# angela000/DQNFlappyBird

Hardware: NVIDIA B200
Metric: env frames/sec (step+render+preproc) (higher is better)
Workload: dtype u8

## Files before the change

### dqnflappybird_b200/csrc/fb_qnet_tc.cu

```cuda
#include <cudaTypedefs.h>

#include <stdlib.h>
#include <string.h>

#include <map>
#include <new>
#include <vector>

#include "fb_qnet.cuh"
#include "fb_pack.cuh"
#include "fb_tc.cuh"
#include "fb_tc_conv.cuh"


namespace {

constexpr int kStages = 4;
constexpr int kMaxKb = 32;
constexpr int kG1 = 21, kP1 = 441;
constexpr int kG2 = 7, kP2 = 49;
constexpr int kThreads = 192;

struct GemmParams {
    int nkb, kper;
// ... 1783 lines not shown
    FinalizeArgs fa{t->part1, t->part2, t->part3, p->s1, p->s2, p->s3, t->bp1, t->bp2, t->bp3, c1, c23, c23, t->hp, t->hb, G, a.loss_out, 1.f / gscale};
    const int n_compact = L.wf1 + (L.total - L.bf1);
    const int nb_fin = (n_compact + 31) / 32;
    tc::pdl_next_launch_plain(t->nopdl & 16);
    FB_CUDA_OK(tc::launch_pdl(finalize_grads_kernel, dim3(nb_fin), dim3(32 * kFinWarps), 0, st, fa, L, a.grads, ad, t->pw[0]));
    if (a.ad.on && a.xch != nullptr) {
        rc = dist_launch_bucket(a.xch, n, 1, const_cast<float *>(a.params), a.ad.m, a.ad.v, t->adam_pow + 2, a.ad.beta1, a.ad.beta2, a.ad.eps,
                                a.ad.grad_scale, st);
        if (rc) return rc;
    }
    if (a.ad.on) FB_CUDA_OK(fork(t->aux3, st));
    if (per_on_side) FB_CUDA_OK(fork(t->aux4, st));
    return FB_OK;
}

bool same_key(const GraphKey &x, const GraphKey &y) { return memcmp(&x, &y, sizeof(GraphKey)) == 0; }

}

int tc_set_format(fb_qnet *n, int f16) {
    TcState *t = n->tc;
    FB_REQUIRE(t != nullptr, "tc_set_format: no tensor-core state");
    f16 = f16 ? 1 : 0;
    if (t->f16 != f16) {
        for (auto &g : t->graphs) destroy_entry(g);
        t->graphs.clear();
        t->plans.clear();
        n->packed_src[0] = n->packed_src[1] = nullptr;
    }
    t->f16 = f16; t->pw[0].f16 = f16; t->pw[1].f16 = f16;
    return FB_OK;
}

int tc_drop_graphs(fb_qnet *n) {
    if (n->tc) { for (auto &g : n->tc->graphs) destroy_entry(g); n->tc->graphs.clear(); }
    return FB_OK;
}

extern "C" int fb_qnet_set_conv1_mode(fb_qnet *n, int mode) {
    FB_REQUIRE(n != nullptr && n->tc != nullptr && mode >= 0 && mode <= 4, "fb_qnet_set_conv1_mode: needs a tensor-core precision and mode 0..4");
    n->tc->conv1_mode = mode;
    for (auto &g : n->tc->graphs) destroy_entry(g);
    n->tc->graphs.clear();
    return FB_OK;
}

extern "C" int fb_qnet_set_fused_backward(fb_qnet *n, int on) {
    FB_REQUIRE(n != nullptr && n->tc != nullptr, "fb_qnet_set_fused_backward: needs FB_PRECISION_BF16");
    n->tc->fuse_bwd = (on & 1) ? 1 : 0;
    n->tc->fuse_fwd = (on & 2) || on == 1 ? 1 : 0;
    return tc_drop_graphs(n);
}

extern "C" int fb_qnet_use_graphs(fb_qnet *n, int enable) {
    FB_REQUIRE(n != nullptr, "fb_qnet_use_graphs: NULL argument");
    if (n->tc) n->tc->use_graph = enable ? 1 : 0;
    return FB_OK;
}

int tc_step(fb_qnet *n, const QnetStep &a, float beta1_power, float beta2_power, cudaStream_t st) {
    TcState *t = n->tc;
    if (a.ad.on) {
        if (t->pow_host[0] != beta1_power || t->pow_host[1] != beta2_power) {
            float *slot = t->pow_pinned + 2 * (t->pow_slot++ & 15);
            slot[0] = beta1_power; slot[1] = beta2_power;
            FB_CUDA_OK(cudaMemcpyAsync(t->adam_pow, slot, 2 * sizeof(float), cudaMemcpyHostToDevice, st));
        }
        t->pow_host[0] = t->pow_host[1] = -1.f;
    }
    GraphKey key;
    memset(&key, 0, sizeof(key));
    memcpy(&key.a, &a, sizeof(a));
    key.a.pro.t = 0; key.a.pro.beta = 0.0;
    key.pack_online = n->packed_src[0] != a.params;
    key.pack_target = a.variant != 0 && n->packed_src[1] != a.target;
    int rc = FB_OK;
    GraphEntry *ge = nullptr;
    if (t->use_graph) {
        for (auto &g : t->graphs) if (same_key(g.key, key)) { ge = &g; break; }
        if (!ge) {
            if (t->graphs.size() >= 8) { for (auto &g : t->graphs) destroy_entry(g); t->graphs.clear(); }
            t->graphs.push_back(GraphEntry{key, 0, nullptr, nullptr, nullptr, nullptr});
            ge = &t->graphs.back();
        }
    }
    if (ge && ge->exec) {
        if (a.pro.replay != nullptr) { rc = replay_patch_nodes(ge->exec, ge->n_sampler, ge->n_gather, a.pro, a.gamma); if (rc) return rc; }
        FB_CUDA_OK(cudaGraphLaunch(ge->exec, st));
    } else if (ge && ge->seen >= 1) {
        cudaGraph_t graph = nullptr;
        FB_CUDA_OK(cudaStreamBeginCapture(t->cap, cudaStreamCaptureModeRelaxed));
        rc = train_step_launch(n, a, key.pack_online, key.pack_target, t->cap);
        cudaError_t ce = cudaStreamEndCapture(t->cap, &graph);
        if (rc) { if (graph) cudaGraphDestroy(graph); return rc; }
        FB_CUDA_OK(ce);
        cudaError_t ie = cudaGraphInstantiate(&ge->exec, graph, 0);
        if (ie == cudaSuccess && a.pro.replay != nullptr) {
            size_t nn = 0;
            cudaGraphGetNodes(graph, nullptr, &nn);
            std::vector<cudaGraphNode_t> nodes(nn);
            if (nn) cudaGraphGetNodes(graph, nodes.data(), &nn);
            for (size_t i = 0; i < nn; i++) {
                cudaGraphNodeType ty;
                if (cudaGraphNodeGetType(nodes[i], &ty) != cudaSuccess || ty != cudaGraphNodeTypeKernel) continue;
                cudaKernelNodeParams kp{};
                if (cudaGraphKernelNodeGetParams(nodes[i], &kp) != cudaSuccess) continue;
                if (replay_is_sampler(kp.func)) ge->n_sampler = nodes[i];
                else if (replay_is_gather(kp.func)) ge->n_gather = nodes[i];
            }
            if (!ge->n_sampler || !ge->n_gather) { cudaGraphExecDestroy(ge->exec); ge->exec = nullptr; ie = cudaErrorUnknown; }
        }
        if (ie == cudaSuccess && a.pro.replay != nullptr) ge->graph = graph;
        else cudaGraphDestroy(graph);
        FB_CUDA_OK(ie);
        FB_CUDA_OK(cudaGraphLaunch(ge->exec, st));
    } else {
        rc = train_step_launch(n, a, key.pack_online, key.pack_target, st);
        if (rc) return rc;
        if (ge) ge->seen++;
    }
    n->packed_src[0] = a.params;
    if (a.variant != 0) n->packed_src[1] = a.target;
    if (a.ad.on && n->packed_src[1] == a.params) n->packed_src[1] = nullptr;
    if (a.ad.on) { t->pow_host[0] = beta1_power * a.ad.beta1; t->pow_host[1] = beta2_power * a.ad.beta2; }
    return FB_OK;
}

extern "C" int fb_debug_tc_kernel(fb_qnet *n, int which, int B, int reps, const float *params_dev, void *stream) {
    FB_REQUIRE(n && n->tc && params_dev && B > 0 && B <= n->max_batch && reps > 0, "fb_debug_tc_kernel: bad argument");
    TcState *t = n->tc;
    TcPlan *p;
    int rc = make_plan(n, B, &p);
    if (rc) return rc;
    cudaStream_t st = (cudaStream_t)stream;
    const QnetLayout &L = n->L;
    const TcWeightMaps &wm = t->wm[0];
    const FwdWs &f = t->ws[0];
    const int H = L.hidden, P1 = B * kP1, P2 = B * kP2;
    for (int r = 0; r < reps; r++) {
        switch (which) {
            case 0: FB_CUDA_OK((launch_tc_conv<32, kSlab1, 1, 4, 6, 1>(p->x2_s[0], wm.w1p, p->conv1, t->n_sms, EpiConv1{f.z1, params_dev + L.b1, P1, t->f16}, st))); break;
            case 1: FB_CUDA_OK((launch_tc_conv<64, kSlab2, 2, 8, 3, 1>(p->p2_s[0], wm.w2p, p->conv2, t->n_sms, EpiGrid7{f.a2, params_dev + L.b2, P2, t->f16}, st))); break;
            case 2: FB_CUDA_OK((launch_tc_conv<64, kSlab3, 1, 9, 4, 1>(p->a2_s[0], wm.w3p, p->conv3, t->n_sms, EpiConv3{f.a3, params_dev + L.b3, P2, t->f16}, st))); break;
            case 3: FB_CUDA_OK((launch_tc_gemm<128, 2>(p->a3_k[0], wm.wf1n, p->fc1, dim3((B + 127) / 128, H / 128, p->sf),
                                                       EpiStoreF32{f.parth, B, H, (size_t)n->max_batch * H}, st))); break;
            case 4: FB_CUDA_OK((launch_tc_wgrad<32, 2, kSlabW1, 1, 6>(p->x2_w, p->dz1_b, p->conv1_w, p->s1, EpiStoreF32{t->part1, 256, 32, (size_t)256 * 32}, st))); break;
            case 5: FB_CUDA_OK((launch_tc_conv<64, kSlab3, 1, 9, 4, 1>(p->dz3_s, wm.w3d, p->conv3_d, t->n_sms, EpiConv3Dgrad{t->dz2, f.a2, P2, t->f16}, st))); break;
            case 6: FB_CUDA_OK((launch_tc_gemm<64, 0>(p->dh1_k, wm.wf1n, p->fc1_d, dim3((B + 127) / 128, kFlat / 64, 1), EpiFc1Dgrad{t->dz3, f.a3, B, t->f16}, st))); break;
            case 7: FB_CUDA_OK((launch_tc_conv1_fused<4, false>(p->x2_s[0], wm.w1p, Conv1FusedParams{g_probe_view, B, params_dev + L.b1, nullptr, f.p2, t->f16}, t->n_sms, st))); break;
            case 8: FB_CUDA_OK((launch_tc_conv1_fused<4, false>(p->x2_s[0], wm.w1p, Conv1FusedParams{g_probe_view, B, params_dev + L.b1, f.z1, f.p2, t->f16}, t->n_sms, st))); break;
            case 9: FB_CUDA_OK((launch_tc_conv1_fused<6, true>(p->x2_s[0], wm.w1p, Conv1FusedParams{g_probe_view, B, params_dev + L.b1, nullptr, f.p2, t->f16}, t->n_sms, st))); break;
            case 10: FB_CUDA_OK((launch_tc_conv1_fused<6, true>(p->x2_s[0], wm.w1p, Conv1FusedParams{g_probe_view, B, params_dev + L.b1, f.z1, f.p2, t->f16}, t->n_sms, st))); break;
            case 11: FB_CUDA_OK((launch_tc_conv1_fused<6, true>(p->x2_s[0], wm.w1p, Conv1FusedParams{g_probe_view, B, params_dev + L.b1, nullptr, nullptr, t->f16}, t->n_sms, st))); break;
            default: FB_REQUIRE(false, "fb_debug_tc_kernel: which must be 0..11");
        }
    }
    return FB_OK;
}

namespace {
__global__ void __launch_bounds__(128) tc_slab_probe_kernel(const __grid_constant__ CUtensorMap mapA, const __grid_constant__ CUtensorMap mapB,
                                                            int shift, uint32_t base_offset, float *d) {
    extern __shared__ uint8_t smem_raw[];
    __shared__ __align__(8) uint64_t bar_full, bar_done;
    __shared__ uint32_t tmem_slot;
    const uint32_t smem = (tc::smem_u32(smem_raw) + 1023u) & ~1023u;
    const int warp = threadIdx.x >> 5, lane = threadIdx.x & 31;
    if (threadIdx.x == 0) { tc::mbar_init(tc::smem_u32(&bar_full), 1); tc::mbar_init(tc::smem_u32(&bar_done), 1); tc::fence_barrier_init(); }
    if (warp == 0) tc::tmem_alloc(tc::smem_u32(&tmem_slot), 64);
    tc::tc_fence_before(); __syncthreads(); tc::tc_fence_after();
    const uint32_t tmem = tmem_slot, sa = smem, sb = smem + 32768;
    if (threadIdx.x == 0) {
        tc::mbar_expect_tx(tc::smem_u32(&bar_full), 32768 + 8192);
        tc::tma_load_2d(sa, &mapA, 0, 0, tc::smem_u32(&bar_full));
        tc::tma_load_2d(sa + 16384, &mapA, 0, 128, tc::smem_u32(&bar_full));
        tc::tma_load_2d(sb, &mapB, 0, 0, tc::smem_u32(&bar_full));
        tc::mbar_wait(tc::smem_u32(&bar_full), 0);
        tc::tc_fence_after();
        constexpr uint32_t idesc = tc::instr_desc_bf16(128, 64, 0, 0);
        for (int k = 0; k < 4; k++) {
            uint64_t ad = tc::smem_desc(sa + shift * 128 + k * 32, 16, 1024, tc::kSwizzle128) | ((uint64_t)(base_offset & 7u) << 49);
            uint64_t bd = tc::smem_desc(sb + k * 32, 16, 1024, tc::kSwizzle128);
            tc::umma_bf16(tmem, ad, bd, idesc, k != 0);
        }
        tc::umma_commit(tc::smem_u32(&bar_done));
    }
    tc::mbar_wait(tc::smem_u32(&bar_done), 0);
    tc::tc_fence_after();
    for (int c0 = 0; c0 < 64; c0 += 16) {
        float v[16];
        tc::tmem_ld16(tmem + ((uint32_t)(warp * 32) << 16) + (uint32_t)c0, v);
        for (int i = 0; i < 16; i++) d[(warp * 32 + lane) * 64 + c0 + i] = v[i];
    }
    tc::tc_fence_before(); __syncthreads();
    if (warp == 0) tc::tmem_dealloc(tmem, 64);
}
}

extern "C" int fb_debug_tc_slab(int shift, int base_offset, const void *a_dev, const void *b_dev, float *d_dev, void *stream) {
    FB_REQUIRE(a_dev && b_dev && d_dev && shift >= 0 && shift <= 128, "fb_debug_tc_slab: bad argument");
    int rc = ensure_encode();
    if (rc) return rc;
    CUtensorMap ma, mb;
    if ((rc = make_map(&ma, (const bf16 *)a_dev, 256, 64, 64, 128))) return rc;
    if ((rc = make_map(&mb, (const bf16 *)b_dev, 64, 64, 64, 64))) return rc;
    FB_CUDA_OK(cudaFuncSetAttribute(tc_slab_probe_kernel, cudaFuncAttributeMaxDynamicSharedMemorySize, 32768 + 8192 + 1024));
    tc_slab_probe_kernel<<<1, 128, 32768 + 8192 + 1024, (cudaStream_t)stream>>>(ma, mb, shift, (uint32_t)base_offset, d_dev);
    FB_CUDA_OK(cudaGetLastError());
    return FB_OK;
}

namespace {
__global__ void __launch_bounds__(128) tc_mma_rate_kernel(int n, int mn_major, int naccs, int iters, int same_operands, long long *cycles) {
    extern __shared__ uint8_t smem_raw[];
    __shared__ __align__(8) uint64_t bar;
    __shared__ uint32_t tmem_slot;
    const uint32_t smem = (tc::smem_u32(smem_raw) + 1023u) & ~1023u;
    const int warp = threadIdx.x >> 5;
    for (int i = threadIdx.x; i < 48 * 1024 / 4; i += 128) reinterpret_cast<uint32_t *>(smem_raw)[i] = 0x3c003c00u;
    if (threadIdx.x == 0) { tc::mbar_init(tc::smem_u32(&bar), 1); tc::fence_barrier_init(); }
    if (warp == 0) tc::tmem_alloc(tc::smem_u32(&tmem_slot), 512);
    tc::fence_proxy_async();
    tc::tc_fence_before(); __syncthreads(); tc::tc_fence_after();
    const uint32_t tmem = tmem_slot;
    if (warp == 1) {
        const uint32_t idesc = tc::instr_desc_bf16(128, n, mn_major, mn_major);
        const uint32_t hi = tc::smem_desc_hi(1024, tc::kSwizzle128);
        const uint32_t a0 = tc::smem_desc_lo(smem, mn_major ? 8192 : 16), b0 = tc::smem_desc_lo(smem + 16384, mn_major ? 8192 : 16);
        const uint32_t step = same_operands ? 0 : (mn_major ? 128 : 2);
        const uint32_t d1 = naccs > 1 ? (uint32_t)n : 0, d2 = naccs > 2 ? 2u * n : 0, d3 = naccs > 3 ? 3u * n : d1;
        uint32_t elected;
        asm volatile("{\n\t.reg .pred p;\n\telect.sync _|p, 0xffffffff;\n\tselp.b32 %0, 1, 0, p;\n\t}" : "=r"(elected));
        long long t0 = clock64();
        for (int i = 0; i < iters; i += 8) {
            if (elected) {
                tc::umma_bf16_lohi(tmem, a0, hi, b0, hi, idesc, 1);
                tc::umma_bf16_lohi(tmem + d1, a0 + step, hi, b0 + step, hi, idesc, 1);
                tc::umma_bf16_lohi(tmem + d2, a0 + 2 * step, hi, b0 + 2 * step, hi, idesc, 1);
                tc::umma_bf16_lohi(tmem + d3, a0 + 3 * step, hi, b0 + 3 * step, hi, idesc, 1);
                tc::umma_bf16_lohi(tmem, a0, hi, b0, hi, idesc, 1);
                tc::umma_bf16_lohi(tmem + d1, a0 + step, hi, b0 + step, hi, idesc, 1);
                tc::umma_bf16_lohi(tmem + d2, a0 + 2 * step, hi, b0 + 2 * step, hi, idesc, 1);
                tc::umma_bf16_lohi(tmem + d3, a0 + 3 * step, hi, b0 + 3 * step, hi, idesc, 1);
            }
            __syncwarp();
        }
        long long t_issue = clock64();
        if (elected) tc::umma_commit(tc::smem_u32(&bar));
        __syncwarp();
        tc::mbar_wait(tc::smem_u32(&bar), 0);
        long long t1 = clock64();
        if (elected) { cycles[0] = t1 - t0; cycles[1] = t_issue - t0; }
    }
    tc::tc_fence_before(); __syncthreads();
    if (warp == 0) tc::tmem_dealloc(tmem, 512);
}
}

extern "C" int fb_debug_tc_mma_rate(int n, int mn_major, int naccs, int iters, int same_operands, long long *cycles_dev, void *stream) {
    FB_REQUIRE(cycles_dev && n >= 16 && n <= 256 && n % 16 == 0 && naccs >= 1 && naccs * n <= 512 && iters > 0, "fb_debug_tc_mma_rate: bad argument");
    FB_CUDA_OK(cudaFuncSetAttribute(tc_mma_rate_kernel, cudaFuncAttributeMaxDynamicSharedMemorySize, 64 * 1024));
    tc_mma_rate_kernel<<<1, 128, 64 * 1024, (cudaStream_t)stream>>>(n, mn_major, naccs, iters, same_operands, cycles_dev);
    FB_CUDA_OK(cudaGetLastError());
    return FB_OK;
}

extern "C" int fb_debug_tc_gemm(int mode, int bn, int M, int N, int K, const void *a_dev, const void *b_dev, float *d_dev,
                                const uint32_t *strides6, void *stream) {
    FB_REQUIRE(a_dev && b_dev && d_dev && (mode == 0 || mode == 1) && (bn == 32 || bn == 64 || bn == 128) && N % bn == 0,
               "fb_debug_tc_gemm: bad argument");
    int rc = ensure_encode();
    if (rc) return rc;
    cudaStream_t st = (cudaStream_t)stream;
    CUtensorMap ma, mb;
    GemmParams g{};
    const bf16 *A = (const bf16 *)a_dev, *Bm = (const bf16 *)b_dev;
    dim3 grid;
    if (mode == 0) {
        FB_REQUIRE(K % 64 == 0 && K / 64 <= kMaxKb, "fb_debug_tc_gemm: K must be a multiple of 64, at most 2048");
        if ((rc = make_map(&ma, A, M, K, 64, 128))) return rc;
        if ((rc = make_map(&mb, Bm, N, K, 64, bn))) return rc;
        set_kmajor(g);
        g.nkb = K / 64;
        for (int k = 0; k < g.nkb; k++) { g.a_rowoff[k] = 0; g.a_col[k] = k * 64; }
        grid = dim3((M + 127) / 128, N / bn, 1);
    } else {
        FB_REQUIRE((M + 127) / 128 <= 16, "fb_debug_tc_gemm: M must be at most 2048 in mode 1");
        if ((rc = make_map(&ma, A, K, M, 64, 64))) return rc;
        if ((rc = make_map(&mb, Bm, K, N, bn == 32 ? 32 : 64, 64))) return rc;
        set_mnmajor(g, bn);
        g.p_total = K; g.klen = (K + 63) / 64 * 64;
        for (int mt = 0; mt < (M + 127) / 128; mt++) for (int i = 0; i < 2; i++) { g.a2_rowoff[mt][i] = 0; g.a2_col[mt][i] = mt * 128 + i * 64; }
        grid = dim3((M + 127) / 128, N / bn, 1);
    }
    if (strides6) { g.lbo_a = strides6[0]; g.sbo_a = strides6[1]; g.kstep_a = strides6[2]; g.lbo_b = strides6[3]; g.sbo_b = strides6[4]; g.kstep_b = strides6[5]; }
    EpiStoreF32 ep{d_dev, M, N, 0};
    cudaError_t e;
    if (mode == 0) e = bn == 32 ? launch_tc_gemm<32, 0>(ma, mb, g, grid, ep, st) : bn == 64 ? launch_tc_gemm<64, 0>(ma, mb, g, grid, ep, st) : launch_tc_gemm<128, 0>(ma, mb, g, grid, ep, st);
    else e = bn == 32 ? launch_tc_gemm<32, 1>(ma, mb, g, grid, ep, st) : bn == 64 ? launch_tc_gemm<64, 1>(ma, mb, g, grid, ep, st) : launch_tc_gemm<128, 1>(ma, mb, g, grid, ep, st);
    FB_CUDA_OK(e);
    return FB_OK;
}
```

### dqnflappybird_b200/csrc/fb_tc_conv.cuh

```cuda
#pragma once
#include "fb_tc.cuh"

namespace {

constexpr int kConvThreads = 192;

constexpr size_t kExclusiveSmem = 116 * 1024;
constexpr size_t exclusive_smem(size_t need) { return need > kExclusiveSmem ? need : kExclusiveSmem; }

struct ConvParams {
    int n_tiles;
    int slab_row0;
    int kb_rowoff[16];
    int kb_half[16];
    int f16;
};

template <int BN, int SLAB_ROWS, int NHALF, int NKB, int S, int T, class EP>
__global__ void __launch_bounds__(kConvThreads, 1) tc_conv_kernel(const __grid_constant__ CUtensorMap mapA,
                                                                   const __grid_constant__ CUtensorMap mapB, const ConvParams g, const EP ep) {
    constexpr uint32_t HALF_BYTES = SLAB_ROWS * 128, STAGE = NHALF * HALF_BYTES, BBLK = BN * 128, B_BYTES = NKB * BBLK;
    static_assert(SLAB_ROWS % 8 == 0 && SLAB_ROWS <= 256, "slab rows: multiple of 8 (1024-byte stage alignment), one TMA box");
    static_assert(S % T == 0 && 2 * T * BN <= 512, "a group of T tiles occupies T consecutive stages and T accumulators of a set");
    extern __shared__ uint8_t smem_raw[];
// ... 118 lines not shown
template <int BN, int SLAB_ROWS, int NHALF, int NKB, int S>
constexpr size_t conv_smem_bytes() { return (size_t)NKB * BN * 128 + (size_t)S * NHALF * SLAB_ROWS * 128 + 1024; }

template <int BN, int SLAB_ROWS, int NHALF, int NKB, int S, int T, class EP>
static cudaError_t launch_tc_conv(const CUtensorMap &ma, const CUtensorMap &mb, const ConvParams &g, int max_ctas, EP ep, cudaStream_t st) {
    static bool configured = false;
    auto kern = tc_conv_kernel<BN, SLAB_ROWS, NHALF, NKB, S, T, EP>;
    constexpr size_t smem = exclusive_smem(conv_smem_bytes<BN, SLAB_ROWS, NHALF, NKB, S>());
    static_assert(smem <= 227 * 1024, "shared memory budget");
    if (!configured) {
        cudaError_t e = cudaFuncSetAttribute(kern, cudaFuncAttributeMaxDynamicSharedMemorySize, (int)smem);
        if (e != cudaSuccess) return e;
        configured = true;
    }
    int grid = g.n_tiles < max_ctas ? g.n_tiles : max_ctas;
    return tc::launch_pdl(kern, dim3(grid), dim3(kConvThreads), smem, st, ma, mb, g, ep);
}

struct WgradParams {
    int p_total, klen;
    int slab_row0;
    int acc_rowoff[8];
    uint32_t acc_lbo[8];
    int f16;
};

template <int BN, int NACC, int SLAB_ROWS, int NHALF, int S, class EP>
__global__ void __launch_bounds__(kConvThreads, 1) tc_wgrad_kernel(const __grid_constant__ CUtensorMap mapA,
                                                                    const __grid_constant__ CUtensorMap mapB, const WgradParams g, const EP ep) {
    constexpr uint32_t HALF_BYTES = SLAB_ROWS * 128, A_BYTES = NHALF * HALF_BYTES, B_BYTES = 64 * BN * 2, STAGE = A_BYTES + B_BYTES;
    constexpr uint32_t B_LAYOUT = BN == 32 ? tc::kSwizzle64 : tc::kSwizzle128;
    constexpr uint32_t B_SBO = BN == 32 ? 512 : 1024, B_KSTEP = BN == 32 ? 1024 : 2048;
    constexpr uint32_t TMEM_COLS = NACC * BN <= 32 ? 32 : NACC * BN <= 64 ? 64 : NACC * BN <= 128 ? 128 : NACC * BN <= 256 ? 256 : 512;
    static_assert(SLAB_ROWS % 8 == 0 && NACC * BN <= 512 && (BN == 32 || BN == 64), "wgrad tile shape");
    extern __shared__ uint8_t smem_raw[];
    __shared__ __align__(8) uint64_t bar_full[S], bar_empty[S], bar_acc;
    __shared__ uint32_t tmem_slot;
    const uint32_t smem = (tc::smem_u32(smem_raw) + 1023u) & ~1023u;
    const int warp = threadIdx.x >> 5, lane = threadIdx.x & 31;
    const int p_begin = blockIdx.x * g.klen;
    const int nkb = (min(g.klen, g.p_total - p_begin) + 63) >> 6;

    if (threadIdx.x == 0) {
        tc::tma_prefetch_desc(&mapA);
        tc::tma_prefetch_desc(&mapB);
        for (int s = 0; s < S; s++) { tc::mbar_init(tc::smem_u32(&bar_full[s]), 1); tc::mbar_init(tc::smem_u32(&bar_empty[s]), 1); }
        tc::mbar_init(tc::smem_u32(&bar_acc), 1);
        tc::fence_barrier_init();
    }
    if (warp == 1) tc::tmem_alloc(tc::smem_u32(&tmem_slot), TMEM_COLS);
    tc::tc_fence_before();
    __syncthreads();
    tc::tc_fence_after();
    const uint32_t tmem = tmem_slot;
    tc::pdl_wait();
    tc::pdl_launch();

    if (warp == 0) {
        const bool leader = tc::elect_one();
        for (int kb = 0; kb < nkb; kb++) {
            const int s = kb % S;
            tc::mbar_wait(tc::smem_u32(&bar_empty[s]), ((kb / S) & 1) ^ 1u);
            if (leader) {
                const uint32_t full = tc::smem_u32(&bar_full[s]), sa = smem + s * STAGE;
                const int p = p_begin + kb * 64;
                tc::mbar_expect_tx(full, STAGE);
#pragma unroll
                for (int h = 0; h < NHALF; h++) tc::tma_load_2d(sa + h * HALF_BYTES, &mapA, h * 64, p + g.slab_row0, full);
                tc::tma_load_2d(sa + A_BYTES, &mapB, 0, p, full);
            }
            __syncwarp();
        }
    } else if (warp == 1) {
        {
            const bool leader = tc::elect_one();
            const uint32_t idesc = tc::instr_desc_16(128, BN, 1, 1, g.f16);
            constexpr uint32_t ahi = tc::smem_desc_hi(1024, tc::kSwizzle128), bhi = tc::smem_desc_hi(B_SBO, B_LAYOUT);
            uint32_t a_lo0[NACC];
#pragma unroll
            for (int a = 0; a < NACC; a++)
                a_lo0[a] = tc::smem_desc_lo(smem + g.acc_rowoff[a] * 128, NHALF == 2 ? HALF_BYTES : g.acc_lbo[a]);
            const uint32_t b_lo0 = tc::smem_desc_lo(smem + A_BYTES, 8192);
            for (int kb = 0; kb < nkb; kb++) {
                const int s = kb % S;
                tc::mbar_wait(tc::smem_u32(&bar_full[s]), (kb / S) & 1);
                tc::tc_fence_after();
                const uint32_t soff = s * (STAGE >> 4);
                if (leader) {
#pragma unroll
                    for (int k = 0; k < 4; k++)
#pragma unroll
                        for (int a = 0; a < NACC; a++)
                            tc::umma_bf16_lohi(tmem + a * BN, a_lo0[a] + soff + k * 128, ahi, b_lo0 + soff + k * (B_KSTEP >> 4), bhi, idesc,
                                               (kb | k) != 0);
                    tc::umma_commit(tc::smem_u32(&bar_empty[s]));
                }
                __syncwarp();
            }
            if (leader) tc::umma_commit(tc::smem_u32(&bar_acc));
            __syncwarp();
        }
    } else {
        const int q = warp & 3;
        tc::mbar_wait(tc::smem_u32(&bar_acc), 0);
        tc::tc_fence_after();
        float4 *stage = reinterpret_cast<float4 *>(smem_raw + (smem - tc::smem_u32(smem_raw))) + q * 256;
        float *outp = ep.out + (size_t)blockIdx.x * ep.split_stride;
#pragma unroll 1
        for (int a = 0; a < NACC; a++)
#pragma unroll 1
            for (int c0 = 0; c0 < BN; c0 += 32) {
                float v[32];
                if (nkb > 0) tc::tmem_ld32(tmem + ((uint32_t)(q * 32) << 16) + (uint32_t)(a * BN + c0), v);
                else {
#pragma unroll
                    for (int i = 0; i < 32; i++) v[i] = 0.f;
                }
#pragma unroll
                for (int j = 0; j < 8; j++)
                    stage[lane * 8 + (j ^ (lane & 7))] = make_float4(v[4 * j] * ep.scale, v[4 * j + 1] * ep.scale, v[4 * j + 2] * ep.scale, v[4 * j + 3] * ep.scale);
                __syncwarp();
#pragma unroll
                for (int j = 0; j < 8; j++) {
                    const int r = (lane >> 3) + 4 * j, c4 = lane & 7, row = a * 128 + q * 32 + r;
                    const float4 x = stage[r * 8 + (c4 ^ (r & 7))];
                    if (row < ep.rows) *reinterpret_cast<float4 *>(outp + (size_t)row * ep.ld + c0 + 4 * c4) = x;
                }
                __syncwarp();
            }
    }
    tc::tc_fence_before();
    __syncthreads();
    if (warp == 1) tc::tmem_dealloc(tmem, TMEM_COLS);
}

template <int BN, int NACC, int SLAB_ROWS, int NHALF, int S, class EP>
static cudaError_t launch_tc_wgrad(const CUtensorMap &ma, const CUtensorMap &mb, const WgradParams &g, int splits, EP ep, cudaStream_t st) {
    static bool configured = false;
    auto kern = tc_wgrad_kernel<BN, NACC, SLAB_ROWS, NHALF, S, EP>;
    constexpr size_t smem = exclusive_smem((size_t)S * (NHALF * SLAB_ROWS * 128 + 64 * BN * 2) + 1024);
    static_assert(smem <= 227 * 1024, "shared memory budget");
    if (!configured) {
        cudaError_t e = cudaFuncSetAttribute(kern, cudaFuncAttributeMaxDynamicSharedMemorySize, (int)smem);
        if (e != cudaSuccess) return e;
        configured = true;
    }
    return tc::launch_pdl(kern, dim3(splits), dim3(kConvThreads), smem, st, ma, mb, g, ep);
}

}

namespace {

constexpr int kBuilders = 256;
constexpr int kRoleThreads1 = 64 + 256;
constexpr int kFusedThreads = kRoleThreads1 + kBuilders;
constexpr int kTileRows1 = 6, kTilePos1 = kTileRows1 * 21;
constexpr int kSlabF = 152;

constexpr int kRawRows = 32, kRawBytes = 4 * kRawRows * 80;
constexpr int kRawStages = 4;

template <int NT>
__device__ __forceinline__ void slab_from_raw(uint8_t *slab, const uint8_t *raw, int tq, int tid, int f16) {
    constexpr int K = (kSlabF * 8 + NT - 1) / NT, LAST = kSlabF * 8 - 1;
    uint32_t t[K][4];
    uint32_t dst[K];
#pragma unroll
    for (int k = 0; k < K; k++) {
        int item = tid + k * NT;
        item = item < LAST ? item : LAST;
        const int r = item >> 3, c16 = item & 7;
        const int bh_l = (r * 3121) >> 16, bw = r - bh_l * 21;
        const int rr = 4 * bh_l + (c16 >> 1), ih = 24 * tq - 2 + rr, iw = 4 * bw - 2 + 2 * (c16 & 1);
        const bool col_ok = (unsigned)iw < 80u;
        const bool valid = col_ok && kTileRows1 * tq + bh_l < 21 && (unsigned)ih < 80u;
        const uint8_t *src = raw + rr * 80 + (col_ok ? iw : 0);
#pragma unroll
        for (int c = 0; c < 4; c++) t[k][c] = *reinterpret_cast<const unsigned short *>(src + c * (kRawRows * 80));
        dst[k] = (uint32_t)(r * 128 + ((c16 ^ (r & 7)) << 4)) | (valid ? 0x80000000u : 0u);
    }
#pragma unroll
    for (int k = 0; k < K; k++) {
        const bool valid = (dst[k] & 0x80000000u) != 0;
        uint32_t w[4];
#pragma unroll
        for (int s2 = 0; s2 < 2; s2++)
#pragma unroll
            for (int h = 0; h < 2; h++) {
                const float lo = (float)((t[k][2 * h] >> (8 * s2)) & 255), hi = (float)((t[k][2 * h + 1] >> (8 * s2)) & 255);
                w[s2 * 2 + h] = valid ? tc::pack2(lo, hi, f16) : 0u;
            }
        if (tid + k * NT <= LAST) *reinterpret_cast<uint4 *>(slab + (dst[k] & 0x7fffffffu)) = make_uint4(w[0], w[1], w[2], w[3]);
    }
}

struct Conv1FusedParams {
    FrameView fv;
    int B;
    const float *bias;
    __nv_bfloat16 *z1;
    __nv_bfloat16 *p2;
    int f16;
};

template <int S, bool FROM_X2>
__global__ void __launch_bounds__(FROM_X2 ? kRoleThreads1 : kFusedThreads, 1) tc_conv1_fused_kernel(const __grid_constant__ CUtensorMap mapA,
                                                                                          const __grid_constant__ CUtensorMap mapB,
                                                                                          const Conv1FusedParams g) {
    constexpr int BN = 32, NKB = 4;
    constexpr uint32_t STAGE = kSlabF * 128, BBLK = BN * 128, B_BYTES = NKB * BBLK, ZS_BYTES = 128 * BN * 2;
    extern __shared__ uint8_t smem_raw[];
    __shared__ __align__(8) uint64_t bar_full[S], bar_empty[S], bar_b, bar_acc_full[2], bar_acc_empty[2], bar_raw_full[kRawStages],
        bar_raw_empty[kRawStages];
    __shared__ uint32_t tmem_slot;
    __shared__ __align__(16) float bias_s[BN];
    uint8_t *smem_gen = smem_raw + ((1024u - (tc::smem_u32(smem_raw) & 1023u)) & 1023u);
    const uint32_t smem_b = tc::smem_u32(smem_gen), smem_a = smem_b + B_BYTES;
    uint8_t *slab_gen = smem_gen + B_BYTES, *zs_gen = slab_gen + S * STAGE, *raw_gen = zs_gen + 4 * ZS_BYTES;
    const int warp = threadIdx.x >> 5, lane = threadIdx.x & 31;
    const int n_tiles = 4 * g.B;
    const long long total_rows = (long long)g.B * 441;

    if (threadIdx.x == 0) {
        tc::tma_prefetch_desc(&mapB);
        for (int s = 0; s < S; s++) { tc::mbar_init(tc::smem_u32(&bar_full[s]), 1); tc::mbar_init(tc::smem_u32(&bar_empty[s]), 1); }
        tc::mbar_init(tc::smem_u32(&bar_b), 1);
        for (int a = 0; a < 2; a++) { tc::mbar_init(tc::smem_u32(&bar_acc_full[a]), 1); tc::mbar_init(tc::smem_u32(&bar_acc_empty[a]), 4); }
        for (int k = 0; k < kRawStages; k++) { tc::mbar_init(tc::smem_u32(&bar_raw_full[k]), 1); tc::mbar_init(tc::smem_u32(&bar_raw_empty[k]), 1); }
        tc::fence_barrier_init();
    }
    if (warp == 1) tc::tmem_alloc(tc::smem_u32(&tmem_slot), 64);
    tc::tc_fence_before();
    __syncthreads();
    tc::tc_fence_after();
    const uint32_t tmem = tmem_slot;
    if (threadIdx.x == 0) {
        tc::mbar_expect_tx(tc::smem_u32(&bar_b), B_BYTES);
        for (int kb = 0; kb < NKB; kb++) tc::tma_load_2d(smem_b + kb * BBLK, &mapB, kb * 64, 0, tc::smem_u32(&bar_b));
    }
    if (threadIdx.x >= 64 && threadIdx.x < 64 + BN) bias_s[threadIdx.x - 64] = g.bias[threadIdx.x - 64];
    tc::pdl_wait();
    tc::pdl_launch();
    __syncthreads();

    if (warp == 0 && FROM_X2) {
        const bool leader = tc::elect_one();
        int i = 0;
        for (int tile = blockIdx.x; tile < n_tiles; tile += gridDim.x, i++) {
            const int s = i % S;
            tc::mbar_wait(tc::smem_u32(&bar_empty[s]), ((i / S) & 1) ^ 1u);
            if (leader) {
                const uint32_t full = tc::smem_u32(&bar_full[s]);
                tc::mbar_expect_tx(full, STAGE);
                tc::tma_load_2d(smem_a + s * STAGE, &mapA, 0, (tile >> 2) * 441 + (tile & 3) * kTilePos1, full);
            }
            __syncwarp();
        }
    } else if (warp == 0) {
        const bool leader = tc::elect_one();
        int i = 0;
        for (int tile = blockIdx.x; tile < n_tiles; tile += gridDim.x, i++) {
            const int rs = i % kRawStages, b = tile >> 2, tq = tile & 3;
            tc::mbar_wait(tc::smem_u32(&bar_raw_empty[rs]), ((i / kRawStages) & 1) ^ 1u);
            if (leader) {
                const int ih0 = 24 * tq - 2, lo = ih0 < 0 ? 0 : ih0, hi = ih0 + kRawRows > 80 ? 80 : ih0 + kRawRows;
                const uint32_t bytes = (uint32_t)(hi - lo) * 80u, full = tc::smem_u32(&bar_raw_full[rs]);
                const uint32_t dst = tc::smem_u32(raw_gen) + rs * kRawBytes + (uint32_t)(lo - ih0) * 80u;
                tc::mbar_expect_tx(full, 4 * bytes);
#pragma unroll
                for (int c = 0; c < 4; c++) tc::bulk_load_1d(dst + c * (kRawRows * 80), g.fv.chan(b, c) + lo * 80, bytes, full);
            }
            __syncwarp();
        }
    } else if (warp >= kRoleThreads1 / 32) {
        constexpr int GT = kBuilders / 2;
        const int grp = (threadIdx.x - kRoleThreads1) / GT, tid = (threadIdx.x - kRoleThreads1) - grp * GT;
        int i = grp;
        for (int tile = blockIdx.x + grp * (int)gridDim.x; tile < n_tiles; tile += 2 * (int)gridDim.x, i += 2) {
            const int s = i % S, rs = i % kRawStages;
            tc::mbar_wait(tc::smem_u32(&bar_raw_full[rs]), (i / kRawStages) & 1);
            tc::mbar_wait(tc::smem_u32(&bar_empty[s]), ((i / S) & 1) ^ 1u);
            slab_from_raw<GT>(slab_gen + s * STAGE, raw_gen + rs * kRawBytes, tile & 3, tid, g.f16);
            tc::fence_proxy_async();
            if (grp == 0) asm volatile("bar.sync 2, %0;" ::"n"(GT) : "memory");
            else asm volatile("bar.sync 3, %0;" ::"n"(GT) : "memory");
            if (tid == 0) { tc::mbar_arrive(tc::smem_u32(&bar_full[s])); tc::mbar_arrive(tc::smem_u32(&bar_raw_empty[rs])); }
        }
    } else if (warp == 1) {
        const bool leader = tc::elect_one();
        const uint32_t idesc = tc::instr_desc_16(128, BN, 0, 0, g.f16);
        constexpr uint32_t dhi = tc::smem_desc_hi(1024, tc::kSwizzle128);
        const uint32_t a_lo0 = tc::smem_desc_lo(smem_a, 16), b_lo0 = tc::smem_desc_lo(smem_b, 16);
        tc::mbar_wait(tc::smem_u32(&bar_b), 0);
        int i = 0;
        for (int tile = blockIdx.x; tile < n_tiles; tile += gridDim.x, i++) {
            const int s = i % S, as = i & 1;
            tc::mbar_wait(tc::smem_u32(&bar_acc_empty[as]), ((i >> 1) & 1) ^ 1u);
            tc::mbar_wait(tc::smem_u32(&bar_full[s]), (i / S) & 1);
            tc::tc_fence_after();
            if (leader) {
                const uint32_t a_lo = a_lo0 + s * (STAGE >> 4);
#pragma unroll
                for (int kb = 0; kb < NKB; kb++) {
                    const uint32_t tap = (uint32_t)(((kb >> 1) * 21 + (kb & 1)) * 128) >> 4;
#pragma unroll
                    for (int k = 0; k < 4; k++)
                        tc::umma_bf16_lohi(tmem + as * BN, a_lo + tap + 2 * k, dhi, b_lo0 + ((kb * BBLK + k * 32) >> 4), dhi, idesc, (kb | k) != 0);
                }
                tc::umma_commit(tc::smem_u32(&bar_empty[s]));
                tc::umma_commit(tc::smem_u32(&bar_acc_full[as]));
            }
            __syncwarp();
        }
    } else if (warp >= 2 && warp < kRoleThreads1 / 32) {
        const int eg = (warp - 2) >> 2;
        const int q = warp & 3, r = q * 32 + lane;
        const int et = threadIdx.x - 64 - 128 * eg;
        int i = eg;
        for (int tile = blockIdx.x + eg * (int)gridDim.x; tile < n_tiles; tile += 2 * (int)gridDim.x, i += 2) {
            const int as = i & 1, b = tile >> 2, tq = tile & 3;
            tc::mbar_wait(tc::smem_u32(&bar_acc_full[as]), (i >> 1) & 1);
            tc::tc_fence_after();
            float v[32];
            tc::tmem_ld32(tmem + ((uint32_t)(q * 32) << 16) + (uint32_t)(as * BN), v);
            tc::tc_fence_before();
            __syncwarp();
            if (lane == 0) tc::mbar_arrive(tc::smem_u32(&bar_acc_empty[as]));
            const int oh_l = r / 21, ow = r - oh_l * 21, oh = kTileRows1 * tq + oh_l;
            const bool ok = r < kTilePos1 && oh < 20 && ow < 20;
            float bia[32];
#pragma unroll
            for (int k = 0; k < 8; k++) {
                const float4 t4 = reinterpret_cast<const float4 *>(bias_s)[k];
                bia[4 * k] = t4.x; bia[4 * k + 1] = t4.y; bia[4 * k + 2] = t4.z; bia[4 * k + 3] = t4.w;
            }
            const float keep = ok ? 1.f : 0.f;
            uint32_t w[16];
#pragma unroll
            for (int k = 0; k < 16; k++) {
                const float x0 = fmaxf(v[2 * k] + bia[2 * k], 0.f) * keep, x1 = fmaxf(v[2 * k + 1] + bia[2 * k + 1], 0.f) * keep;
                w[k] = tc::pack2(x0, x1, g.f16);
            }
            uint4 *zs = reinterpret_cast<uint4 *>(zs_gen + (i & 3) * ZS_BYTES + r * 64);
            if (g.p2 != nullptr)
#pragma unroll
            for (int k = 0; k < 4; k++) zs[(k + (r >> 1)) & 3] = make_uint4(w[4 * k], w[4 * k + 1], w[4 * k + 2], w[4 * k + 3]);
            if (ok && g.z1 != nullptr) {
                uint4 *d = reinterpret_cast<uint4 *>(g.z1 + ((size_t)b * 441 + oh * 21 + ow) * BN);
#pragma unroll
                for (int k = 0; k < 4; k += 2)
                    tc::st_global_256(d + k, make_uint4(w[4 * k], w[4 * k + 1], w[4 * k + 2], w[4 * k + 3]), make_uint4(w[4 * k + 4], w[4 * k + 5], w[4 * k + 6], w[4 * k + 7]));
            }
            if (g.p2 == nullptr) continue;
            if (eg == 0) asm volatile("bar.sync 1, 128;" ::: "memory");
            else asm volatile("bar.sync 4, 128;" ::: "memory");
            if (et < 120) {
                const int ph_l = et / 40, rem = et - ph_l * 40, pw = rem >> 2, cg = rem & 3, ph = 3 * tq + ph_l;
                if (ph < 10) {
                    const uint8_t *zb = zs_gen + (i & 3) * ZS_BYTES;
                    auto ld = [&](int row) { return *reinterpret_cast<const uint4 *>(zb + row * 64 + (((cg + (row >> 1)) & 3) << 4)); };
                    const int r0 = (2 * ph_l) * 21 + 2 * pw;
                    uint4 m = ld(r0), o1 = ld(r0 + 1), o2 = ld(r0 + 21), o3 = ld(r0 + 22);
                    uint32_t *pm = reinterpret_cast<uint32_t *>(&m);
                    const uint32_t *p1 = reinterpret_cast<const uint32_t *>(&o1), *p2 = reinterpret_cast<const uint32_t *>(&o2),
                                   *p3 = reinterpret_cast<const uint32_t *>(&o3);
#pragma unroll
                    for (int k = 0; k < 4; k++) pm[k] = tc::max2(tc::max2(pm[k], p1[k], g.f16), tc::max2(p2[k], p3[k], g.f16), g.f16);
                    const int bh = (ph + 1) >> 1, rr = (ph + 1) & 1, bw = (pw + 1) >> 1, ss = (pw + 1) & 1;
                    *reinterpret_cast<uint4 *>(g.p2 + ((size_t)b * 49 + bh * 7 + bw) * 128 + rr * 64 + ss * 32 + cg * 8) = m;
                }
            }
        }
    }
    tc::tc_fence_before();
    __syncthreads();
    if (warp == 1) tc::tmem_dealloc(tmem, 64);
}

template <int S, bool FROM_X2>
static cudaError_t launch_tc_conv1_fused(const CUtensorMap &ma, const CUtensorMap &mb, const Conv1FusedParams &g, int max_ctas, cudaStream_t st) {
    static bool configured = false;
    auto kern = tc_conv1_fused_kernel<S, FROM_X2>;
    constexpr size_t smem = exclusive_smem(4 * 32 * 128 + (size_t)S * kSlabF * 128 + 4 * 128 * 32 * 2 + (FROM_X2 ? 0 : kRawStages * kRawBytes) + 1024);
    if (!configured) {
        cudaError_t e = cudaFuncSetAttribute(kern, cudaFuncAttributeMaxDynamicSharedMemorySize, (int)smem);
        if (e != cudaSuccess) return e;
        configured = true;
    }
    int grid = 4 * g.B < max_ctas ? 4 * g.B : max_ctas;
    return tc::launch_pdl(kern, dim3(grid), dim3(FROM_X2 ? kRoleThreads1 : kFusedThreads), smem, st, ma, mb, g);
}

}
```

Measured before the change: 848.6 million.

## Rebuild conv1 input slabs with vectorized row loads and shuffle-based im2col

The builder path that expands raw u8 frames into the swizzled conv1 operand slab is rewritten. It now uses five warps that each load 16-byte row chunks, borrow neighbouring bytes with warp shuffles and funnel shifts, and convert u8 to half with a byte_perm magic-number trick instead of per-element float conversion. The builder thread count rises from 256 to 320 to match, and the pooled-activation staging buffer gets an extra row swizzle to cut shared-memory bank conflicts. A debug probe case for a fused conv2/conv3 kernel is also added. The goal is less instruction and shared-memory overhead in slab construction, at the cost of more threads per block and stricter layout assumptions.

Measured after the change: 852.0 million (median of 6 runs). Within noise of the previous version (+0.4%).

```diff
diff --git a/dqnflappybird_b200/csrc/fb_qnet_tc.cu b/dqnflappybird_b200/csrc/fb_qnet_tc.cu
--- a/dqnflappybird_b200/csrc/fb_qnet_tc.cu
+++ b/dqnflappybird_b200/csrc/fb_qnet_tc.cu
@@ -1959,7 +1959,9 @@
             case 9: FB_CUDA_OK((launch_tc_conv1_fused<6, true>(p->x2_s[0], wm.w1p, Conv1FusedParams{g_probe_view, B, params_dev + L.b1, nullptr, f.p2, t->f16}, t->n_sms, st))); break;
             case 10: FB_CUDA_OK((launch_tc_conv1_fused<6, true>(p->x2_s[0], wm.w1p, Conv1FusedParams{g_probe_view, B, params_dev + L.b1, f.z1, f.p2, t->f16}, t->n_sms, st))); break;
             case 11: FB_CUDA_OK((launch_tc_conv1_fused<6, true>(p->x2_s[0], wm.w1p, Conv1FusedParams{g_probe_view, B, params_dev + L.b1, nullptr, nullptr, t->f16}, t->n_sms, st))); break;
-            default: FB_REQUIRE(false, "fb_debug_tc_kernel: which must be 0..11");
+            case 12: FB_CUDA_OK((launch_tc_fwd23<2>(p->p2_s[0], wm.w2p, wm.w3p, Fwd23Params{(B + 1) / 2, B, params_dev + L.b2, params_dev + L.b3, nullptr, f.a3, t->f16},
+                                                    t->n_sms, st))); break;
+            default: FB_REQUIRE(false, "fb_debug_tc_kernel: which must be 0..12");
         }
     }
     return FB_OK;
diff --git a/dqnflappybird_b200/csrc/fb_tc_conv.cuh b/dqnflappybird_b200/csrc/fb_tc_conv.cuh
--- a/dqnflappybird_b200/csrc/fb_tc_conv.cuh
+++ b/dqnflappybird_b200/csrc/fb_tc_conv.cuh
@@ -294,7 +294,7 @@
 
 namespace {
 
-constexpr int kBuilders = 256;
+constexpr int kBuilders = 320;
 constexpr int kRoleThreads1 = 64 + 256;
 constexpr int kFusedThreads = kRoleThreads1 + kBuilders;
 constexpr int kTileRows1 = 6, kTilePos1 = kTileRows1 * 21;
@@ -303,38 +303,60 @@
 constexpr int kRawRows = 32, kRawBytes = 4 * kRawRows * 80;
 constexpr int kRawStages = 4;
 
+template <uint32_t SEL>
+__device__ __forceinline__ uint32_t u8x2_to_16(uint32_t x, int f16) {
+    const uint32_t w = __byte_perm(x, 0x64646464u, SEL);
+    __half2 h = __hsub2(*reinterpret_cast<const __half2 *>(&w), __halves2half2(__ushort_as_half(0x6400), __ushort_as_half(0x6400)));
+    if (f16) return *reinterpret_cast<uint32_t *>(&h);
+    const float2 f = __half22float2(h);
+    return tc::pack2(f.x, f.y, 0);
+}
+
+__device__ __forceinline__ void slab_block(uint8_t *slab, int r, int rr, const uint32_t (&lo)[4], const uint32_t (&hi)[4], int f16) {
+    if (r >= kSlabF) return;
+    uint32_t p[4];
+#pragma unroll
+    for (int f = 0; f < 4; f++) p[f] = __funnelshift_r(lo[f], hi[f], 16);
+    const uint32_t x01 = __byte_perm(p[0], p[1], 0x5140), x23 = __byte_perm(p[2], p[3], 0x5140);
+    const uint32_t y01 = __byte_perm(p[0], p[1], 0x7362), y23 = __byte_perm(p[2], p[3], 0x7362);
+    const uint4 c0 = make_uint4(u8x2_to_16<0x4140>(x01, f16), u8x2_to_16<0x4140>(x23, f16), u8x2_to_16<0x4342>(x01, f16), u8x2_to_16<0x4342>(x23, f16));
+    const uint4 c1 = make_uint4(u8x2_to_16<0x4140>(y01, f16), u8x2_to_16<0x4140>(y23, f16), u8x2_to_16<0x4342>(y01, f16), u8x2_to_16<0x4342>(y23, f16));
+    *reinterpret_cast<uint4 *>(slab + r * 128 + (((2 * rr) ^ (r & 7)) << 4)) = c0;
+    *reinterpret_cast<uint4 *>(slab + r * 128 + (((2 * rr + 1) ^ (r & 7)) << 4)) = c1;
+}
+
 template <int NT>
 __device__ __forceinline__ void slab_from_raw(uint8_t *slab, const uint8_t *raw, int tq, int tid, int f16) {
-    constexpr int K = (kSlabF * 8 + NT - 1) / NT, LAST = kSlabF * 8 - 1;
-    uint32_t t[K][4];
-    uint32_t dst[K];
-#pragma unroll
-    for (int k = 0; k < K; k++) {
-        int item = tid + k * NT;
-        item = item < LAST ? item : LAST;
-        const int r = item >> 3, c16 = item & 7;
-        const int bh_l = (r * 3121) >> 16, bw = r - bh_l * 21;
-        const int rr = 4 * bh_l + (c16 >> 1), ih = 24 * tq - 2 + rr, iw = 4 * bw - 2 + 2 * (c16 & 1);
-        const bool col_ok = (unsigned)iw < 80u;
-        const bool valid = col_ok && kTileRows1 * tq + bh_l < 21 && (unsigned)ih < 80u;
-        const uint8_t *src = raw + rr * 80 + (col_ok ? iw : 0);
-#pragma unroll
-        for (int c = 0; c < 4; c++) t[k][c] = *reinterpret_cast<const unsigned short *>(src + c * (kRawRows * 80));
-        dst[k] = (uint32_t)(r * 128 + ((c16 ^ (r & 7)) << 4)) | (valid ? 0x80000000u : 0u);
-    }
-#pragma unroll
-    for (int k = 0; k < K; k++) {
-        const bool valid = (dst[k] & 0x80000000u) != 0;
-        uint32_t w[4];
-#pragma unroll
-        for (int s2 = 0; s2 < 2; s2++)
-#pragma unroll
-            for (int h = 0; h < 2; h++) {
-                const float lo = (float)((t[k][2 * h] >> (8 * s2)) & 255), hi = (float)((t[k][2 * h + 1] >> (8 * s2)) & 255);
-                w[s2 * 2 + h] = valid ? tc::pack2(lo, hi, f16) : 0u;
-            }
-        if (tid + k * NT <= LAST) *reinterpret_cast<uint4 *>(slab + (dst[k] & 0x7fffffffu)) = make_uint4(w[0], w[1], w[2], w[3]);
-    }
+    static_assert(NT == 5 * 32 && kRawRows == 32, "five warps: rows x words 0..3, then word 4");
+    const int lane = tid & 31, warp = tid >> 5;
+    const int g = warp < 4 ? lane >> 3 : 4, R = warp < 4 ? 8 * warp + (lane & 7) : lane;
+    const int bh = R >> 2, rr = R & 3, ih = 24 * tq - 2 + R, r0 = 21 * bh + 4 * g;
+    const bool row_ok = kTileRows1 * tq + bh < 21 && (unsigned)ih < 80u;
+    const uint8_t *src = raw + R * 80 + g * 16;
+    uint4 x[4];
+    uint32_t prev[4];
+#pragma unroll
+    for (int f = 0; f < 4; f++) {
+        x[f] = *reinterpret_cast<const uint4 *>(src + f * (kRawRows * 80));
+        if (!row_ok) x[f] = make_uint4(0, 0, 0, 0);
+    }
+    if (warp < 4) {
+#pragma unroll
+        for (int f = 0; f < 4; f++) {
+            prev[f] = __shfl_up_sync(0xffffffffu, x[f].w, 8);
+            if (g == 0) prev[f] = 0;
+        }
+    } else {
+#pragma unroll
+        for (int f = 0; f < 4; f++) prev[f] = row_ok ? *reinterpret_cast<const uint32_t *>(src - 4 + f * (kRawRows * 80)) : 0u;
+    }
+    const uint32_t w0[4] = {x[0].x, x[1].x, x[2].x, x[3].x}, w1[4] = {x[0].y, x[1].y, x[2].y, x[3].y};
+    const uint32_t w2[4] = {x[0].z, x[1].z, x[2].z, x[3].z}, w3[4] = {x[0].w, x[1].w, x[2].w, x[3].w}, zero[4] = {0, 0, 0, 0};
+    slab_block(slab, r0, rr, prev, w0, f16);
+    slab_block(slab, r0 + 1, rr, w0, w1, f16);
+    slab_block(slab, r0 + 2, rr, w1, w2, f16);
+    slab_block(slab, r0 + 3, rr, w2, w3, f16);
+    if (warp == 4) slab_block(slab, r0 + 4, rr, w3, zero, f16);
 }
 
 struct Conv1FusedParams {
@@ -484,7 +506,7 @@
                 const float x0 = fmaxf(v[2 * k] + bia[2 * k], 0.f) * keep, x1 = fmaxf(v[2 * k + 1] + bia[2 * k + 1], 0.f) * keep;
                 w[k] = tc::pack2(x0, x1, g.f16);
             }
-            uint4 *zs = reinterpret_cast<uint4 *>(zs_gen + (i & 3) * ZS_BYTES + r * 64);
+            uint4 *zs = reinterpret_cast<uint4 *>(zs_gen + (i & 3) * ZS_BYTES + (r ^ ((r >> 1) & 1)) * 64);
             if (g.p2 != nullptr)
 #pragma unroll
             for (int k = 0; k < 4; k++) zs[(k + (r >> 1)) & 3] = make_uint4(w[4 * k], w[4 * k + 1], w[4 * k + 2], w[4 * k + 3]);
@@ -501,7 +523,7 @@
                 const int ph_l = et / 40, rem = et - ph_l * 40, pw = rem >> 2, cg = rem & 3, ph = 3 * tq + ph_l;
                 if (ph < 10) {
                     const uint8_t *zb = zs_gen + (i & 3) * ZS_BYTES;
-                    auto ld = [&](int row) { return *reinterpret_cast<const uint4 *>(zb + row * 64 + (((cg + (row >> 1)) & 3) << 4)); };
+                    auto ld = [&](int row) { return *reinterpret_cast<const uint4 *>(zb + (row ^ ((row >> 1) & 1)) * 64 + (((cg + (row >> 1)) & 3) << 4)); };
                     const int r0 = (2 * ph_l) * 21 + 2 * pw;
                     uint4 m = ld(r0), o1 = ld(r0 + 1), o2 = ld(r0 + 21), o3 = ld(r0 + 22);
                     uint32_t *pm = reinterpret_cast<uint32_t *>(&m);
```
